# 3dimaging/rasr

Measured on AMD Instinct MI355X. Metric: frames/sec scored, 39-dim x 800k-density diag-GMM, higher is better.
Workload: dtype f32 (operands split into 2 f16 pieces, 3 f16 MFMA products, f32 accumulate); 1 GPU; 800k-density diag-GMM, 39-dim, diagonal-maximum, batched frames; scorer=diagonal-maximum, mixtures=5000, densities_per_mixture=160, covariance_tying=pooled, dimension=39, frames_per_launch=32768, parallelism=frame-sharded replicas x1

## Files before the change

include/rasr_gmm.h:

```cpp
#ifndef RASR_GMM_H
#define RASR_GMM_H

#include <stddef.h>
#include <stdint.h>

#ifdef __cplusplus
extern "C" {
#endif

#define GMM_OK 0
#define GMM_ERR_INVALID_ARGUMENT -1
#define GMM_ERR_UNSUPPORTED -2
#define GMM_ERR_DEVICE -3
#define GMM_ERR_OUT_OF_MEMORY -4
#define GMM_ERR_CAPACITY -5

typedef enum {
    GMM_BATCH_DIAGONAL_MAXIMUM_FLOAT = 0,
    GMM_BATCH_PRESELECTION_FLOAT     = 1,
    GMM_BATCH_PRESELECTION_INT       = 2,
    GMM_BATCH_DIAGONAL_MAXIMUM_INT   = 3,
    GMM_BATCH_DIAGONAL_MAXIMUM_FAST  = 4,
    GMM_DIAGONAL_MAXIMUM             = 5,
    GMM_SIMD_DIAGONAL_MAXIMUM        = 9,
// ... 26 lines not shown
    uint32_t clusters;
    uint32_t select_clusters;
    uint32_t clustering_iterations;
    float    backoff_score;
    const char* cache_archive;
} gmm_scorer_config;

#define GMM_FLAG_NATIVE_F32 1u
#define GMM_FLAG_SPLIT_TILE16 2u
#define GMM_FLAG_SPLIT_TILE32 4u
#define GMM_FLAG_REFERENCE_ORDER 8u
#define GMM_FLAG_FULL_KEYS 16u
#define GMM_FLAG_NO_SCORE_ONLY_TWIN 32u
#define GMM_FLAG_CACHE_ARCHIVE_READ_ONLY 64u
#define GMM_FLAG_ACCEPT_SPREAD_BOUND 128u

typedef struct gmm_scorer gmm_scorer;

void gmm_default_config(gmm_scorer_config* cfg);

int gmm_scorer_create(const gmm_mixture_set* mixture_set, gmm_scorer_type type,
                      const gmm_scorer_config* config, int device, gmm_scorer** out);
int gmm_scorer_destroy(gmm_scorer* scorer);

uint32_t gmm_scorer_n_mixtures(const gmm_scorer* scorer);
uint32_t gmm_scorer_dimension(const gmm_scorer* scorer);
uint32_t gmm_scorer_n_covariances(const gmm_scorer* scorer);
int      gmm_scorer_type_of(const gmm_scorer* scorer);

int gmm_score_device(gmm_scorer* scorer, const float* frames, uint32_t n_frames, uint32_t frame_stride,
// ... 43 lines not shown
                              double* log_z, double* minimum_score, uint32_t* minimum_index, uint32_t* n_active);

int gmm_host_alloc(size_t bytes, void** ptr);
int gmm_host_free(void* ptr);

int gmm_scorer_quantization(const gmm_scorer* scorer, float* scaling, float* inverse_quantization_factor);

int gmm_scorer_multiply_and_quantize(const gmm_scorer* scorer, const float* feature, uint8_t* out);

int gmm_prepare_quantized_host(const gmm_mixture_set* mixture_set, gmm_scorer_type type, float* scaling,
                               float* isv, float* log_norm, uint8_t* prepared_mean, int32_t* constant_weight);

int gmm_scorer_launch_info(const gmm_scorer* scorer, uint32_t n_frames, uint32_t* n_launches,
                           const char** main_kernel_name);

int gmm_scorer_k_steps(const gmm_scorer* scorer, uint32_t* k_steps);

int gmm_float_spread_bound(const gmm_mixture_set* mixture_set, gmm_scorer_type type, const gmm_scorer_config* config,
                           double* statistic, double* predicted);
int gmm_scorer_spread_bound(const gmm_scorer* scorer, double* statistic, double* predicted);

int gmm_scorer_set_timing(gmm_scorer* scorer, int enable);
int gmm_scorer_kernel_time(gmm_scorer* scorer, double* total_ms, uint32_t* n_launches, int reset);

#define GMM_CLUSTERING_BUILT 0
#define GMM_CLUSTERING_WRITTEN 1
#define GMM_CLUSTERING_CACHED 2
int gmm_scorer_clustering_source(const gmm_scorer* scorer, int* source);
int gmm_cache_archive_read_item(const char* path, const char* name, void* data, uint64_t capacity, uint64_t* size);
int gmm_cache_archive_write_item(const char* path, const char* name, const void* data, uint64_t size);
// ... 31 lines not shown
```

rasr_amd/_capi.py:

```python
from __future__ import annotations

import ctypes
import os

_HERE = os.path.dirname(os.path.abspath(__file__))
LIB_PATH = os.environ.get("RASR_GMM_LIB") or os.path.join(_HERE, "lib", "librasr_gmm.so")

GMM_OK = 0
GMM_ERR_INVALID_ARGUMENT = -1
GMM_ERR_UNSUPPORTED = -2
GMM_ERR_DEVICE = -3
GMM_ERR_OUT_OF_MEMORY = -4
GMM_ERR_CAPACITY = -5
GMM_ESTIMATOR_CHUNK = 512
STATE_POSTERIOR_CHUNK = 256
DEFAULT_WEIGHT_THRESHOLD = 2.0 ** -23
GMM_FLAG_NATIVE_F32 = 1
GMM_FLAG_SPLIT_TILE16 = 2
GMM_FLAG_SPLIT_TILE32 = 4
GMM_FLAG_REFERENCE_ORDER = 8
GMM_FLAG_FULL_KEYS = 16
GMM_FLAG_NO_SCORE_ONLY_TWIN = 32
GMM_FLAG_CACHE_ARCHIVE_READ_ONLY = 64
GMM_FLAG_ACCEPT_SPREAD_BOUND = 128
FLOAT_CONTRACT = 1e-4
GMM_CLUSTERING = {0: "built", 1: "written", 2: "cached"}

BATCH_DIAGONAL_MAXIMUM_FLOAT = 0
BATCH_PRESELECTION_FLOAT = 1
BATCH_PRESELECTION_INT = 2
BATCH_DIAGONAL_MAXIMUM_INT = 3
BATCH_DIAGONAL_MAXIMUM_FAST = 4
DIAGONAL_MAXIMUM = 5
SIMD_DIAGONAL_MAXIMUM = 9
DIAGONAL_SUM = 12

SCORER_TYPES = {
    "batch-diagonal-maximum-float": BATCH_DIAGONAL_MAXIMUM_FLOAT,
    "batch-diagonal-maximum-int": BATCH_DIAGONAL_MAXIMUM_INT,
# ... 97 lines not shown
      ctypes.c_double, ctypes.c_void_p, ctypes.c_void_p, ctypes.c_uint32, ctypes.c_void_p, ctypes.c_void_p,
      ctypes.c_void_p, ctypes.c_void_p, ctypes.c_void_p]),
    ("gmm_state_posteriors_host", ctypes.c_int,
     [ctypes.c_void_p, ctypes.c_void_p, ctypes.c_uint32, ctypes.c_uint32, ctypes.c_void_p, ctypes.c_double,
      ctypes.c_double, ctypes.c_void_p, ctypes.c_void_p, ctypes.c_uint32, ctypes.c_void_p, ctypes.c_void_p,
      ctypes.c_void_p, ctypes.c_void_p]),
    ("gmm_host_alloc", ctypes.c_int, [ctypes.c_size_t, ctypes.POINTER(ctypes.c_void_p)]),
    ("gmm_host_free", ctypes.c_int, [ctypes.c_void_p]),
    ("gmm_scorer_quantization", ctypes.c_int, [ctypes.c_void_p, _f32p, _f32p]),
    ("gmm_scorer_multiply_and_quantize", ctypes.c_int, [ctypes.c_void_p, ctypes.c_void_p, ctypes.c_void_p]),
    ("gmm_prepare_quantized_host", ctypes.c_int,
     [ctypes.POINTER(MixtureSetDesc), ctypes.c_int, _f32p, ctypes.c_void_p, ctypes.c_void_p, ctypes.c_void_p,
      ctypes.c_void_p]),
    ("gmm_scorer_launch_info", ctypes.c_int,
     [ctypes.c_void_p, ctypes.c_uint32, _u32p, ctypes.POINTER(ctypes.c_char_p)]),
    ("gmm_scorer_k_steps", ctypes.c_int, [ctypes.c_void_p, _u32p]),
    ("gmm_float_spread_bound", ctypes.c_int,
     [ctypes.POINTER(MixtureSetDesc), ctypes.c_int, ctypes.POINTER(ScorerConfig), _f64p, _f64p]),
    ("gmm_scorer_spread_bound", ctypes.c_int, [ctypes.c_void_p, _f64p, _f64p]),
    ("gmm_scorer_set_timing", ctypes.c_int, [ctypes.c_void_p, ctypes.c_int]),
    ("gmm_scorer_kernel_time", ctypes.c_int,
     [ctypes.c_void_p, ctypes.POINTER(ctypes.c_double), _u32p, ctypes.c_int]),
    ("gmm_scorer_density_clustering", ctypes.c_int,
     [ctypes.c_void_p, _u32p, _u32p, ctypes.c_void_p, ctypes.c_void_p]),
    ("gmm_scorer_cluster_selection", ctypes.c_int, [ctypes.c_void_p, ctypes.c_uint32, ctypes.c_void_p]),
    ("gmm_scorer_clustering_source", ctypes.c_int, [ctypes.c_void_p, ctypes.POINTER(ctypes.c_int)]),
    ("gmm_cache_archive_read_item", ctypes.c_int,
     [ctypes.c_char_p, ctypes.c_char_p, ctypes.c_void_p, ctypes.c_uint64, ctypes.POINTER(ctypes.c_uint64)]),
    ("gmm_cache_archive_write_item", ctypes.c_int, [ctypes.c_char_p, ctypes.c_char_p, ctypes.c_void_p, ctypes.c_uint64]),
    ("gmm_density_clustering_seeds", ctypes.c_int, [ctypes.c_uint32, ctypes.c_uint32, _u32p]),
# ... 93 lines not shown
```

rasr_amd/csrc/gmm_kernels.hh:

```
#pragma once

#include <hip/hip_runtime.h>

#include <cstdint>
#include <mutex>
#include <set>
#include <type_traits>
#include <utility>

namespace rasr_gmm {

enum class Kernel { I8Seg, I8Cls, I8Presel, Direct, SplitPair, SplitWide, SplitPresel, Split32, SplitSum, Split32Sum, F32 };
constexpr bool isSplitKernel(Kernel k) {
    return k == Kernel::SplitPair || k == Kernel::SplitWide || k == Kernel::SplitPresel || k == Kernel::Split32 ||
           k == Kernel::SplitSum || k == Kernel::Split32Sum;
}

template <int... N, class F>
bool dispatchInt(uint32_t v, std::integer_sequence<int, N...>, F&& f) {
    return ((v == uint32_t(N) ? (f(std::integral_constant<int, N>{}), true) : false) || ...);
}

inline hipError_t allowDynamicLds(const void* fn, int bytes) {
    static std::mutex                        mu;
// ... 84 lines not shown
#ifndef GMM_SPLIT_FPB
#define GMM_SPLIT_FPB 256
#endif
constexpr uint32_t kSplitFramesPerBlock = GMM_SPLIT_FPB;
constexpr uint32_t kSplitWaves          = kSplitFramesPerBlock / 64;
constexpr uint32_t kSplitMainWaves      = kSplitFramesPerBlock / (16 * kSplitNF);
#ifndef GMM_SPLIT_WIDE
#define GMM_SPLIT_WIDE 1
#endif
constexpr uint32_t splitWideFrames(uint32_t ks) {
    return GMM_SPLIT_WIDE && ks <= 4 ? 256u : 0u;
}

constexpr uint32_t kSplitWideChunkTiles = (1u << 22) / 5u - 16u;

constexpr uint32_t kSplitLimbs   = 4;
constexpr uint32_t kSplitXXLimbs = 3;
constexpr int kSplitXXExp[kSplitXXLimbs] = {15, 4, -7};
inline uint32_t splitKSteps(uint32_t dimension) {
    return (3 * dimension + kSplitLimbs + kSplitXXLimbs + 31) / 32;
}
inline uint32_t splitKSteps32(uint32_t dimension) {
    return (3 * dimension + kSplitLimbs + kSplitXXLimbs + 15) / 16;
}
inline uint32_t splitCovKSteps(uint32_t dimension) {
    return (6 * dimension + kSplitLimbs + 31) / 32;
}

struct SplitArgs {
    const void*     tileH;
// ... 3 lines not shown
    const float*    frameXX;
    const int32_t*  frameExp;
    float*          scores;
    uint32_t*       best;
    uint32_t        nFrames, nFramesPad, scoreStride;
    uint32_t        nChunks, nFrameTiles, mixBase;
    int             flavor;
    uint32_t        tileBits;
    float           offsetK0;
    float           outScale;
    const uint32_t* selT;
    const void*     tileClu;
    uint32_t        nClusters;
    int             presel;
    float           backoff;
};

hipError_t launchPrepareFramesI8(const float* frames, uint32_t nFrames, uint32_t frameStride, uint32_t nFramesPad,
                                 uint32_t nFramesRead, uint32_t D, uint32_t C, uint32_t KS, const float* isv, int8_t* frameQ,
                                 int32_t* frameSS, hipStream_t stream);
hipError_t launchPrepareFramesF32(const float* frames, uint32_t nFrames, uint32_t frameStride, uint32_t nFramesPad,
                                  uint32_t nFramesRead, uint32_t D, uint32_t C, uint32_t KS, int foldNorm, const float* isv,
                                  const float* centre, float* frameX,
                                  float* frameXX, hipStream_t stream);
hipError_t launchPrepareFramesSplit(const float* frames, uint32_t nFrames, uint32_t frameStride, uint32_t nFramesRead,
                                    uint32_t D, uint32_t rows, uint32_t kSteps, const float* isv, const float* centre,
                                    const float* dimScale,
                                    const int32_t* limbExp, void* frameH, float* frameXX, int32_t* frameExp,
                                    hipStream_t stream);
hipError_t launchPrepareFramesSplitCov(const float* frames, uint32_t nFrames, uint32_t frameStride, uint32_t nFramesRead,
// ... 120 lines not shown
```

rasr_amd/csrc/gmm_kernels_i8.hip:

```cpp
#include <type_traits>

#include "gmm_device.hh"

#ifndef GMM_I8_SLOTS
#define GMM_I8_SLOTS 1
#endif

namespace rasr_gmm {
namespace dev {

__global__ __launch_bounds__(256) void prepareFramesI8(const float* __restrict__ frames, uint32_t nFrames,
                                                        uint32_t frameStride, uint32_t nFramesPad,
                                                        uint32_t nFramesRead, uint32_t D,
                                                        uint32_t C, uint32_t KS, const float* __restrict__ isv,
                                                        int8_t* __restrict__ frameQ, int32_t* __restrict__ frameSS) {
    const uint32_t g = blockIdx.x * 8u + (threadIdx.x >> 5), blk = threadIdx.x & 31u;
    if (g >= C * nFramesRead)
        return;
    const uint32_t c = g / nFramesRead, f = g % nFramesRead;
    const float*   x  = frames + static_cast<size_t>(f) * frameStride;
    const float*   iv = isv + static_cast<size_t>(c) * KS * 64;
    i32x4*         out = reinterpret_cast<i32x4*>(frameQ + (static_cast<size_t>(c) * nFramesPad + f) * KS * 64);
    int            ss = 0;
    if (blk < KS * 4) {
// ... 1089 lines not shown
        if constexpr (KS == 1) {
            if (a.scoreOnly == 2) {
                constexpr int NFC = (W == 4 && NF == kI8NF) ? kI8ClsNF : NF;
                hipLaunchKernelGGL((dev::scoreI8Cls<NFC, kSeg, W>), dim3(grid), dim3(64 * W), 0, s, a, a.mixTileOff,
                                   a.scores, a.mixOddMask);
                return;
            }
            if (a.scoreOnly) {
                hipLaunchKernelGGL((dev::scoreI8Seg<NF, 1, false, kSeg, true, W>), dim3(grid), dim3(64 * W), 0, s, a,
                                   a.mixTileOff, a.scores, nullptr, a.mixOddMask);
                return;
            }
        }
        hipLaunchKernelGGL((dev::scoreI8Seg<NF, KS, false, kSeg, false, W>), dim3(grid), dim3(64 * W), 0, s, a,
                           a.mixTileOff, a.scores, a.best, nullptr);
        return;
    }
    hipLaunchKernelGGL((dev::scoreI8<NF, KS, MULTI>), dim3(grid), dim3(256), 0, s, a);
}

hipError_t launchScoreI8(const I8Args& a, uint32_t kSteps, bool multiCov, hipStream_t stream) {
    const uint32_t grid = 8u * ((a.nChunks + 7u) / 8u) * a.nFrameTiles;
    if (grid == 0)
        return hipSuccess;
    if (a.presel && (multiCov || a.nClusters == 0 || a.nClusters > 256 || !a.selT || !a.tileClu ||
                     (kI8PreselNF == 8 && !a.selC)))
        return hipErrorInvalidValue;
    if (a.scoreOnly && (multiCov || kSteps != 1 || !a.mixOddMask))
        return hipErrorInvalidValue;
    if (a.smallTile && a.presel)
        return hipErrorInvalidValue;
    if (kSteps == 1 && a.smallTile == 2 && !multiCov)
        launchI8T<4, 1, false, 1>(a, grid, stream);
// ... 17 lines not shown
```

rasr_amd/csrc/gmm_kernels_split.hip:

```cpp
#include "gmm_device.hh"

#include <type_traits>
#include <utility>

#ifndef GMM_SPLIT_MIN_WAVES
#define GMM_SPLIT_MIN_WAVES 1
#endif
#ifndef GMM_SPLIT_IL
#define GMM_SPLIT_IL 24
#endif
#ifndef GMM_SPLIT_PRESEL_NF
#define GMM_SPLIT_PRESEL_NF 8
#endif
constexpr int splitPreselNF(int ks) { return GMM_SPLIT_PRESEL_NF == 8 && ks <= 5 ? 8 : 4; }
#ifndef GMM_SPLIT_PF
#define GMM_SPLIT_PF 2
#endif
#ifndef GMM_SPLIT_SUM_NF
#define GMM_SPLIT_SUM_NF 4
#endif

namespace rasr_gmm {
namespace dev {

// ... 503 lines not shown
                }
            }
        });
    }
}

#ifndef GMM_SPLIT_WIDE_PF
#define GMM_SPLIT_WIDE_PF 3
#endif
#ifndef GMM_SPLIT_WIDE_IL
#define GMM_SPLIT_WIDE_IL 64
#endif
#define GMM_WIDE_ROW_RSRC(ptr) \
    __builtin_amdgcn_make_buffer_rsrc((ptr) + rowOff, (short)0, static_cast<int>(a.nFrames * 4u), 0x00020000)

template <int KS, bool BEST>
__global__ __launch_bounds__(64, 1) void scoreSplitWide(SplitArgs a, const uint32_t* __restrict__ mixTileOff) {
    constexpr uint32_t FPB = splitWideFrames(KS);
    constexpr int      NF = FPB / 16, NH = NF / 4, PF = GMM_SPLIT_WIDE_PF, U = PF % 2 == 0 ? PF : 2 * PF;
    static_assert(FPB == 256, "16 column blocks: the frame operands fill the accumulator file, four frames per lane");
    const int      lane = threadIdx.x & 63;
    const uint32_t g    = static_cast<uint32_t>(lane) >> 4;
    uint32_t       chunk, ft;
    if (!mapBlock(a.nChunks, a.nFrameTiles, chunk, ft))
        return;
    const uint32_t frame0 = ft * FPB, fb0 = frame0 / 16u;
    const uint32_t m0 = a.chunkMixOff[chunk], m1 = a.chunkMixOff[chunk + 1];
    const uint32_t T0 = mixTileOff[m0], T1 = mixTileOff[m1];

    const auto     tileRsrc = __builtin_amdgcn_make_buffer_rsrc(
            const_cast<char*>(static_cast<const char*>(a.tileH)) + static_cast<size_t>(T0) * (KS * 1024u), (short)0,
            static_cast<int>((T1 - T0 + PF) * (KS * 1024u)), 0x00020000);
    const uint32_t laneOff  = static_cast<uint32_t>(lane) * 16u;
    const auto     loadTile = [&](uint32_t tt, f16x8(&A)[KS]) __attribute__((always_inline)) {
        const uint32_t so = (tt - T0) * (KS * 1024u);
#pragma unroll
        for (int s = 0; s < KS; ++s)
            A[s] = __builtin_bit_cast(f16x8, __builtin_amdgcn_raw_buffer_load_b128(tileRsrc, laneOff + 1024u * s, so, 0));
    };
    const f16x8*   fh = static_cast<const f16x8*>(a.frameH);
// ... 17 lines not shown
            asm volatile("" : "+a"(B[cb][s]));
#pragma unroll
    for (int h = 0; h < NH; ++h)
        asm volatile("" ::"v"(eOut[h]));

    f16x8 R[PF][KS];
#pragma unroll
    for (int j = 0; j < PF; ++j)
        loadTile(T0 + j, R[j]);

    const uint32_t kmask = BEST ? (1u << a.tileBits) - 1u : 0u;
    uint32_t       vmask = ~kmask;
    asm volatile("" : "+v"(vmask));
    const float noneScore = __fmul_rn(a.outScale, a.flavor == 2 ? 0.5f * 3.40282347e+38f : 3.40282347e+38f);

    uint32_t   best[NF][2];
    const auto resetBest = [&]() {
#pragma unroll
        for (int cb = 0; cb < NF; ++cb)
            best[cb][0] = best[cb][1] = 0xffffffffu;
    };
    const auto chain = [&](const f16x8(&A)[KS], f32x4(&acc)[NF]) __attribute__((always_inline)) {
#pragma unroll
        for (int cb = 0; cb < NF; ++cb)
            acc[cb] = f32x4{0.0f, 0.0f, 0.0f, 0.0f};
#pragma unroll
        for (int s = 0; s < KS; ++s)
#pragma unroll
            for (int cb = 0; cb < NF; ++cb)
                acc[cb] = __builtin_amdgcn_mfma_f32_16x16x32_f16(A[s], B[cb][s], acc[cb], 0, 0, 0);
    };
    uint32_t   tag[4] = {0u, 1u, 2u, 3u};
    const auto epilogue = [&](const f32x4(&acc)[NF]) __attribute__((always_inline)) {
#pragma unroll
        for (int r = 0; r < 4; ++r)
            asm("" : "+s"(tag[r]));
#pragma unroll
        for (int cb = 0; cb < NF; ++cb) {
            uint32_t v[4];
#pragma unroll
            for (int r = 0; r < 4; ++r)
                v[r] = BEST ? (__float_as_uint(acc[cb][r]) & vmask) | tag[r] : __float_as_uint(acc[cb][r]);
            best[cb][0] = umin3(umin3(best[cb][0], v[0], v[1]), v[2], v[3]);
        }
#pragma unroll
        for (int r = 0; r < 4; ++r)
            tag[r] += 4u;
    };

    uint32_t   m = m0, tEnd = m0 < m1 ? mixTileOff[m0 + 1] : T0;
    uint32_t tNxt  = mixTileOff[min(m0 + 2u, m1)];
    size_t rowOff  = static_cast<size_t>(m0 - a.mixBase) * a.scoreStride;
    const auto nextMixture = [&](uint32_t tNext) __attribute__((always_inline)) {
        ++m;
        rowOff += a.scoreStride;
        tEnd = m < m1 ? tNxt : tNext;
        tNxt = mixTileOff[min(m + 2u, m1)];
    };
    const auto emit = [&]() __attribute__((always_inline)) {
        uint32_t key[NH], idx[NH];
        float    score[NH];
#pragma unroll
        for (int h = 0; h < NH; ++h) {
            uint32_t k[4], grp;
#pragma unroll
            for (int cb = 0; cb < 4; ++cb)
                k[cb] = min(best[4 * h + cb][0], best[4 * h + cb][1]);
            reduceKeysSplit<BEST>(k, key[h], grp);
            idx[h] = (((key[h] & kmask & ~3u) | grp) << 2) | (key[h] & 3u);
        }
        finalizeSplit<BEST, NH>(a, key, kmask, eOut, noneScore, score, idx);
        const uint32_t off = (frame0 + NH * static_cast<uint32_t>(lane)) * 4u;
        __builtin_amdgcn_raw_buffer_store_b128(u32x4{__float_as_uint(score[0]), __float_as_uint(score[1]),
                                                     __float_as_uint(score[2]), __float_as_uint(score[3])},
                                               GMM_WIDE_ROW_RSRC(a.scores), off, 0, GMM_STORE_CPOL);
        if constexpr (BEST)
            __builtin_amdgcn_raw_buffer_store_b128(u32x4{idx[0], idx[1], idx[2], idx[3]}, GMM_WIDE_ROW_RSRC(a.best), off, 0,
                                                   GMM_STORE_CPOL);
    };
    const auto advance = [&](uint32_t tNext) __attribute__((always_inline)) {
        nextMixture(tNext);
        while (m < m1 && tEnd == tNext) {
// ... 2 lines not shown
        }
    };
    const auto finish = [&](uint32_t tNext) __attribute__((always_inline)) {
        if (__builtin_expect(tNext == tEnd, 0)) {
            emit();
            resetBest();
            advance(tNext);
#pragma unroll
            for (int r = 0; r < 4; ++r)
                tag[r] &= 3u;
        }
    };
    constexpr int  kIl   = GMM_SPLIT_WIDE_IL * NF / 16;
    constexpr int  kIlE  = 3 * NF;
    constexpr bool kTail = kIl >= kIlE && kIlE + KS + 4 <= NF * KS;
    const auto    step = [&](const f16x8(&A)[KS], f32x4(&cur)[NF], const f32x4(&prev)[NF]) __attribute__((always_inline)) {
        chain(A, cur);
        epilogue(prev);
#pragma unroll
        for (int i = 0; i < (kTail ? kIlE : kIl); ++i) {
            __builtin_amdgcn_sched_group_barrier(0x008, 1, 0);
            __builtin_amdgcn_sched_group_barrier(0x002, 2, 0);
        }
        if constexpr (kTail) {
#pragma unroll
            for (int i = 0; i < KS; ++i) {
                __builtin_amdgcn_sched_group_barrier(0x008, 1, 0);
                __builtin_amdgcn_sched_group_barrier(0x020, 1, 0);
            }
#pragma unroll
            for (int i = 0; i < 4; ++i) {
                __builtin_amdgcn_sched_group_barrier(0x008, 1, 0);
                __builtin_amdgcn_sched_group_barrier(0x004, 2, 0);
            }
            __builtin_amdgcn_sched_group_barrier(0x008, NF * KS - kIlE - KS - 4, 0);
        }
        else
            __builtin_amdgcn_sched_group_barrier(0x008, NF * KS - kIl, 0);
    };

    resetBest();
    while (m < m1 && tEnd == T0) {
        emit();
        nextMixture(T0);
    }
    if (T0 < T1) {
        f32x4 acc[2][NF];
        chain(R[0], acc[0]);
        loadTile(T0 + PF, R[0]);
        uint32_t t = T0 + 1;
        const auto sub = [&](auto ic, uint32_t tt) __attribute__((always_inline)) {
            constexpr int i = decltype(ic)::value, set = (1 + i) % PF, cur = (1 + i) % 2, prv = i % 2;
            step(R[set], acc[cur], acc[prv]);
            loadTile(tt + PF, R[set]);
            finish(tt);
        };
        for (; t + U <= T1; t += U)
            staticFor<U>([&](auto ic) __attribute__((always_inline)) { sub(ic, t + decltype(ic)::value); });
        bool live = true;
        staticFor<U>([&](auto ic) __attribute__((always_inline)) {
            constexpr int  i  = decltype(ic)::value;
            const uint32_t tt = t + i;
            if (live) {
                if (tt < T1) {
                    sub(ic, tt);
// ... 738 lines not shown
}

hipError_t launchPrepareFramesSplitCov(const float* frames, uint32_t nFrames, uint32_t frameStride, uint32_t nFramesRead,
                                       uint32_t D, uint32_t kSteps, const float* centre, const float* dimScale,
                                       const int32_t* limbExp, void* frameH, int32_t* frameExp, hipStream_t stream) {
    hipLaunchKernelGGL(dev::prepareFramesSplitCov, dim3((nFramesRead + 7) / 8), dim3(256), 0, stream, frames, nFrames,
                       frameStride, nFramesRead, D, kSteps, centre, dimScale, limbExp, static_cast<dev::u32x4*>(frameH),
                       frameExp);
    return hipGetLastError();
}

template <int KS>
static void launchSplitK(const SplitArgs& a, Kernel kernel, uint32_t grid, hipStream_t s) {
    if constexpr (splitWideFrames(KS) != 0) {
        if (kernel == Kernel::SplitWide) {
            hipLaunchKernelGGL((a.best ? dev::scoreSplitWide<KS, true> : dev::scoreSplitWide<KS, false>), dim3(grid), dim3(64),
                               0, s, a, a.mixTileOff);
            return;
        }
    }
    if (kernel == Kernel::SplitPresel) {
        const uint32_t lds = kSplitFramesPerBlock / 64u * a.nClusters * 64u;
        (void)allowDynamicLds(reinterpret_cast<const void*>(&dev::scoreSplit<KS, false, true>),
                              static_cast<int>(kSplitFramesPerBlock / 64u * 256u * 64u));
        hipLaunchKernelGGL((dev::scoreSplit<KS, false, true>), dim3(grid), dim3(kSplitFramesPerBlock / splitPreselNF(KS) * 4),
                           lds, s, a, a.mixTileOff);
    }
    else
        hipLaunchKernelGGL((a.best ? dev::scoreSplit<KS, true, false> : dev::scoreSplit<KS, false, false>), dim3(grid),
                           dim3(64 * kSplitMainWaves), 0, s, a, a.mixTileOff);
}

// ... 12 lines not shown
template <int KS>
static void launchSplit32SumK(const SplitArgs& a, uint32_t grid, hipStream_t s) {
    hipLaunchKernelGGL((a.best ? dev::scoreSplit32Sum<KS, true> : dev::scoreSplit32Sum<KS, false>), dim3(grid),
                       dim3(64 * (kSplitFramesPerBlock / 128)), 0, s, a, a.mixTileOff);
}

using KSteps16 = std::integer_sequence<int, 8, 7, 6, 5, 4, 3, 2, 1>;
using KSteps32 = std::integer_sequence<int, 10, 9, 8, 7, 6, 5, 4, 3, 2, 1>;

hipError_t launchScoreSplit(const SplitArgs& a, Kernel kernel, uint32_t kSteps16, hipStream_t stream) {
    const uint32_t grid = 8u * ((a.nChunks + 7u) / 8u) * a.nFrameTiles;
    if (grid == 0)
        return hipSuccess;
    if ((a.presel != 0) != (kernel == Kernel::SplitPresel) ||
        (a.presel && (a.nClusters == 0 || a.nClusters > 256 || !a.selT || !a.tileClu)) ||
        (kernel == Kernel::SplitWide && splitWideFrames(kSteps16) == 0))
        return hipErrorInvalidValue;
    bool ok = false;
    switch (kernel) {
        case Kernel::Split32:
            ok = dispatchInt(kSteps16, KSteps32{}, [&](auto ks) { launchSplit32K<decltype(ks)::value>(a, grid, stream); });
            break;
        case Kernel::SplitPair:
        case Kernel::SplitWide:
        case Kernel::SplitPresel:
            ok = dispatchInt(kSteps16, KSteps16{}, [&](auto ks) { launchSplitK<decltype(ks)::value>(a, kernel, grid, stream); });
            break;
        case Kernel::Split32Sum:
            ok = dispatchInt(kSteps16, KSteps32{}, [&](auto ks) { launchSplit32SumK<decltype(ks)::value>(a, grid, stream); });
            break;
        case Kernel::SplitSum:
// ... 9 lines not shown
```

rasr_amd/csrc/gmm_score.cc:

```cpp
#include <algorithm>
#include <cstdlib>

#include "gmm_scorer.hh"

namespace rasr_gmm {


KernelPlan kernelPlanOf(const gmm_scorer& s) {
    const bool presel = isPreselection(s.type);
    KernelPlan p;
    p.launches = presel ? 3 : 2;
    if (const auto* q = s.quantized()) {
        p.kernel = presel ? Kernel::I8Presel : (q->scoreOnly == kScoreOnlySlots ? Kernel::I8Cls : Kernel::I8Seg);
        p.framesPerBlock = presel ? kI8PreselFramesPerBlock
                                  : (p.kernel == Kernel::I8Cls ? kI8ClsFramesPerBlock : kI8FramesPerBlock);
        p.smallTiles     = !presel;
        p.name           = "scoreI8";
    }
    else if (std::holds_alternative<DirectModel>(s.model))
        p = {Kernel::Direct, kDirectFramesPerBlock, false, p.launches, "scoreDirect"};
    else if (const auto* m = std::get_if<SplitModel>(&s.model)) {
        const bool     rows32 = m->splitRows == 32;
        const uint32_t wide   = splitWideFrames(m->kSteps16);
        p.framesPerBlock      = kSplitFramesPerBlock;
// ... 31 lines not shown
    return p;
}

int waitAsync(gmm_scorer* s) {
    if (!s->host.asyncCall)
        return GMM_OK;
    s->host.asyncCall  = 0;
    const hipError_t e = hipEventSynchronize(s->host.asyncDone.get());
    if (e != hipSuccess)
        return fail(GMM_ERR_DEVICE, std::string("hipEventSynchronize (GMM_HOST_ASYNC call): ") + hipGetErrorString(e));
    return GMM_OK;
}

namespace {

int chunkTableFor(gmm_scorer* s, uint32_t nFrameTiles, const ChunkTable** out) {
    auto it = s->chunks.find(nFrameTiles);
    if (it != s->chunks.end()) {
        *out = &it->second;
        return GMM_OK;
    }
#ifndef GMM_TARGET_BLOCKS
#define GMM_TARGET_BLOCKS 8192
#endif
#ifndef GMM_SPLIT_TARGET_BLOCKS
#define GMM_SPLIT_TARGET_BLOCKS 2048
#endif
    static const uint32_t kOverride = [] {
        const char* e = std::getenv("RASR_GMM_TARGET_BLOCKS");
        const long  v = e ? std::strtol(e, nullptr, 10) : 0;
        return v > 0 ? static_cast<uint32_t>(v) : 0u;
    }();
    const Kernel   k       = s->plan.kernel;
    const uint32_t kTargetBlocks =
            kOverride ? kOverride
            : isSplitKernel(k) ? std::clamp<uint32_t>(nFrameTiles * 256u, 1024u,
                                             k == Kernel::SplitSum ? uint32_t(GMM_TARGET_BLOCKS)
                                                                   : uint32_t(GMM_SPLIT_TARGET_BLOCKS))
            : k == Kernel::I8Seg || k == Kernel::I8Cls ? std::clamp<uint32_t>(nFrameTiles * 1024u, 2048u, uint32_t(GMM_TARGET_BLOCKS))
                                                       : uint32_t(GMM_TARGET_BLOCKS);
    uint32_t target = std::max<uint32_t>(1, (kTargetBlocks + nFrameTiles - 1) / nFrameTiles);
    if (target > 8)
        target = (target + 7u) / 8u * 8u;
    target                  = std::min<uint32_t>(target, std::max<uint32_t>(1, s->nMix));
    uint32_t perChunk = std::max<uint32_t>(1, (s->nTiles + target - 1) / target);
    const uint32_t chunkCap = k == Kernel::SplitWide ? kSplitWideChunkTiles : 0xffffffffu;
    perChunk                = std::min(perChunk, chunkCap / 2u);
    std::vector<uint32_t> off{0};
    uint32_t              acc = 0;
    for (uint32_t m = 0; m < s->nMix; ++m) {
        acc += s->mixTileOff[m + 1] - s->mixTileOff[m];
        if (acc > chunkCap)
            return fail(GMM_ERR_CAPACITY, "a mixture has more tiles than a scoreSplitWide chunk can address");
        if (acc >= perChunk && m + 1 < s->nMix) {
            off.push_back(m + 1);
            acc = 0;
        }
    }
    off.push_back(s->nMix);
    ChunkTable ct;
    ct.nChunks = static_cast<uint32_t>(off.size() - 1);
    int rc     = upload(ct.dMixOff, off);
    if (rc != GMM_OK)
        return rc;
    *out = &s->chunks.emplace(nFrameTiles, std::move(ct)).first->second;
    return GMM_OK;
}

struct TimedSpan {
    gmm_scorer* s;
    hipStream_t stream;
    hipEvent_t  e = nullptr;
    hipError_t begin() {
        if (!s->timing)
            return hipSuccess;
        if (s->eventsUsed == s->events.size()) {
            std::pair<Event, Event> ev;
            hipError_t              err = ev.first.create();
// ... 122 lines not shown
    a.tileH       = m.dTileH.get();
    a.frameH      = m.dFrameH.get();
    a.frameXX     = m.dFrameXX.get();
    a.frameExp    = m.dFrameExp.get();
    a.best        = s.flavor != Flavor::BatchFloat ? c.best : nullptr;
    a.flavor      = s.flavor == Flavor::DiagonalMaximum ? 2 : (s.flavor == Flavor::DiagonalSum ? 4 : 3);
    a.tileBits    = m.keyBits;
    a.offsetK0    = m.offsetK0;
    a.presel      = c.plan.kernel == Kernel::SplitPresel ? 1 : 0;
    if (s.presel) {
        a.selT      = s.presel->dSelT.get();
        a.tileClu   = s.presel->dTileClu.get();
        a.nClusters = s.presel->clustering.nClusters;
    }
    a.backoff = s.cfg.backoff_score;
    return launchScoreSplit(a, c.plan.kernel, m.kSteps16, c.stream);
}

hipError_t prepareFrames(const gmm_scorer& s, const F32Model& m, const Call& c) {
    return launchPrepareFramesF32(c.frames, c.nFrames, c.frameStride, s.nFramesPad, c.plan.nFramesRead, s.D, s.C, m.kSteps,
                                  m.foldNorm ? 1 : 0, s.dIsv.get(), m.dCentre.get(), m.dFrameX.get(), m.dFrameXX.get(),
                                  c.stream);
}

hipError_t launch(const gmm_scorer& s, const F32Model& m, const Call& c) {
    F32Args a = argsOf<F32Args>(s, c);
    a.tileA       = static_cast<const float*>(m.dTileA.get());
    a.tileCov     = m.dTileCov.get();
    a.rowDns      = m.dRowDns.get();
    a.frameX      = m.dFrameX.get();
    a.frameXX     = m.dFrameXX.get();
// ... 44 lines not shown

int gmm_score_device(gmm_scorer* s, const float* frames, uint32_t nFrames, uint32_t frameStride, float* scores,
                     uint32_t* best, uint32_t scoreStride, void* stream) {
    if (!s)
        return fail(GMM_ERR_INVALID_ARGUMENT, "null scorer");
    const int wrc = waitAsync(s);
    if (wrc != GMM_OK)
        return wrc;
    return scoreImpl(s, frames, nFrames, frameStride, scores, best, scoreStride, static_cast<hipStream_t>(stream));
}

int gmm_scorer_launch_info(const gmm_scorer* s, uint32_t nFrames, uint32_t* nLaunches, const char** name) {
    if (!s)
        return fail(GMM_ERR_INVALID_ARGUMENT, "null scorer");
    s = modelOf(s);
    (void)nFrames;
    if (nLaunches)
        *nLaunches = s->plan.launches;
    if (name)
        *name = s->plan.name;
    return GMM_OK;
}

int gmm_scorer_k_steps(const gmm_scorer* s, uint32_t* kSteps) {
    if (!s || !kSteps)
        return fail(GMM_ERR_INVALID_ARGUMENT, "null scorer or output");
    s = modelOf(s);
    if (const auto* q = s->quantized())
        *kSteps = q->kSteps;
    else if (const auto* m = std::get_if<SplitModel>(&s->model))
        *kSteps = m->kSteps16;
    else if (const auto* f = std::get_if<F32Model>(&s->model))
        *kSteps = f->kSteps;
    else if (const auto* d = std::get_if<DirectModel>(&s->model))
        *kSteps = (d->L - 4u) / 4u;
// ... 7 lines not shown
```

rasr_amd/csrc/gmm_scorer.hh:

```
#pragma once

#include <hip/hip_runtime.h>

#include <map>
#include <memory>
#include <string>
#include <type_traits>
#include <utility>
#include <variant>
#include <vector>

#include "../../include/rasr_gmm.h"
#include "gmm_hostio.hh"
#include "gmm_kernels.hh"
#include "gmm_prepare.hh"
#include "gmm_presel.hh"

namespace rasr_gmm {

void setLastError(const std::string& msg);

inline int fail(int code, const std::string& msg) {
    setLastError(msg);
    return code;
// ... 77 lines not shown
    uint32_t    launches       = 2;
    const char* name           = "scoreF32";
};

struct LaunchPlan {
    Kernel   kernel;
    uint32_t framesPerBlock;
    int      smallTile;
    uint32_t nFrameTiles, nFramesRead;
};


struct ChunkTable {
    uint32_t               nChunks = 0;
    DeviceBuffer<uint32_t> dMixOff;
};

struct QuantizedModel {
    uint32_t kSteps = 0, idxBits = 1, paddedDimension = 0;
    int      scoreOnly = kScoreOnlyNone;
    float    scaling = 0, scalingSquared = 0, invQ = 0, batchScale = 0;
    std::vector<float>     isvScaled;
    DeviceBuffer<void>     dTileA, dTileP;
    DeviceBuffer<uint32_t> dTileCov, dMixOddMask;
    DeviceBuffer<int8_t>   dFrameQ;
    DeviceBuffer<int32_t>  dFrameSS;
};

struct SplitModel {
    uint32_t kSteps16 = 0;
// ... 88 lines not shown
    using Flavor = rasr_gmm::Flavor;
    gmm_scorer_type   type;
    Flavor            flavor;
    int               device = 0;
    gmm_scorer_config cfg{};
    uint32_t          D = 0, C = 0, nMix = 0, mixBase = 0;
    uint32_t          nMixSet = 0;
    uint32_t          nTiles = 0;
    uint32_t          nFramesPad = 0;
    double            spreadStat = 0, spreadPredicted = 0;
    std::vector<uint32_t>            mixTileOff;
    rasr_gmm::DeviceBuffer<uint32_t> dMixTileOff;
    rasr_gmm::DeviceBuffer<float>    dIsv;
    rasr_gmm::KernelPlan             plan;
    std::map<uint32_t, rasr_gmm::ChunkTable> chunks;
    bool                                                   timing = false;
    std::vector<std::pair<rasr_gmm::Event, rasr_gmm::Event>> events;
    size_t                                                 eventsUsed = 0;
    std::variant<std::monostate, rasr_gmm::QuantizedModel, rasr_gmm::SplitModel, rasr_gmm::F32Model,
                 rasr_gmm::DirectModel>
            model;
    std::unique_ptr<rasr_gmm::Preselection> presel;
    std::unique_ptr<rasr_gmm::PairTables>   pairs;
    std::unique_ptr<rasr_gmm::StateScratch> state;
    rasr_gmm::HostPipeline                  host;
    std::unique_ptr<rasr_gmm::DensityGroup, rasr_gmm::DensityGroupDelete> group;
    std::unique_ptr<gmm_scorer> scoresOnly;
    std::string cacheArchive;

    const rasr_gmm::QuantizedModel* quantized() const { return std::get_if<rasr_gmm::QuantizedModel>(&model); }
// ... 39 lines not shown
```

rasr_amd/scorer.py:

```python
from __future__ import annotations

import ctypes
import os

import numpy as np

from . import _capi
from .mixture_set import MixtureSet


def _type_id(t) -> int:
    if isinstance(t, str):
        return _capi.SCORER_TYPES[t]
    return int(t)


def default_config() -> _capi.ScorerConfig:
    cfg = _capi.ScorerConfig()
    _capi.load_library().gmm_default_config(ctypes.byref(cfg))
    return cfg


class Scorer:

    def __init__(self, mixture_set: MixtureSet, scorer_type="SIMD-diagonal-maximum", max_frames: int = 4096,
                 device: int = 0, mixture_weight_scale: float = 1.0, gaussian_scale: float = 1.0,
                 score_scale: float = 1.0, mixture_range: tuple[int, int] | None = None, native_f32: bool = False,
                 split_tile16: bool = False, split_tile32: bool = False, clusters: int = 256,
                 select_clusters: int = 32, clustering_iterations: int = 5, backoff_score: float = 40000.0,
                 reference_order: bool = False, devices=None, exchange: str = "auto", full_keys: bool = False,
                 no_score_only_twin: bool = False, cache_archive: str | None = None,
                 cache_archive_read_only: bool = False, accept_spread_bound: bool = False):
        self._lib = _capi.load_library()
        self.mixture_set = mixture_set
        self.type = _type_id(scorer_type)
        cfg = default_config()
        cfg.max_frames = int(max_frames)
        cfg.mixture_weight_scale = mixture_weight_scale
        cfg.gaussian_scale = gaussian_scale
        cfg.score_scale = score_scale
        if native_f32:
            cfg.flags |= _capi.GMM_FLAG_NATIVE_F32
        if split_tile16:
            cfg.flags |= _capi.GMM_FLAG_SPLIT_TILE16
        if split_tile32:
            cfg.flags |= _capi.GMM_FLAG_SPLIT_TILE32
        if reference_order:
            cfg.flags |= _capi.GMM_FLAG_REFERENCE_ORDER
        if full_keys:
            cfg.flags |= _capi.GMM_FLAG_FULL_KEYS
        if no_score_only_twin:
            cfg.flags |= _capi.GMM_FLAG_NO_SCORE_ONLY_TWIN
        if accept_spread_bound:
            cfg.flags |= _capi.GMM_FLAG_ACCEPT_SPREAD_BOUND
        cfg.clusters = int(clusters)
        cfg.select_clusters = int(select_clusters)
        cfg.clustering_iterations = int(clustering_iterations)
        cfg.backoff_score = float(backoff_score)
        self._cache_archive = None if cache_archive is None else os.fsencode(cache_archive)
        cfg.cache_archive = self._cache_archive
        if cache_archive_read_only:
            cfg.flags |= _capi.GMM_FLAG_CACHE_ARCHIVE_READ_ONLY
        if mixture_range is not None:
            cfg.mixture_begin, cfg.mixture_end = int(mixture_range[0]), int(mixture_range[1])
        self.max_frames = int(max_frames)
        self._mixture_range = ((int(cfg.mixture_begin), int(cfg.mixture_end)) if cfg.mixture_end
                            else (0, int(len(mixture_set.mixture_offsets)) - 1))
        self._desc = mixture_set.desc()
        h = ctypes.c_void_p()
# ... 23 lines not shown
        try:
            self.close()
        except Exception:
            pass

    @property
    def handle(self):
        return self._h

    def main_kernel(self) -> str:
        n = ctypes.c_uint32()
        name = ctypes.c_char_p()
        _capi.check(self._lib.gmm_scorer_launch_info(self._h, 1, ctypes.byref(n), ctypes.byref(name)),
                    "gmm_scorer_launch_info")
        return name.value.decode()

    def k_steps(self) -> int:
        k = ctypes.c_uint32()
        _capi.check(self._lib.gmm_scorer_k_steps(self._h, ctypes.byref(k)), "gmm_scorer_k_steps")
        return k.value

    def spread_bound(self) -> tuple[float, float]:
        st, pr = ctypes.c_double(), ctypes.c_double()
        _capi.check(self._lib.gmm_scorer_spread_bound(self._h, ctypes.byref(st), ctypes.byref(pr)),
                    "gmm_scorer_spread_bound")
        return st.value, pr.value

    def density_clustering(self):
        n = ctypes.c_uint32()
        dp = ctypes.c_uint32()
# ... 309 lines not shown
```

Baseline: 7.989 million frames/s.

## Specialize split-wide kernel for chunks with uniform per-mixture tile counts

```diff
diff --git a/include/rasr_gmm.h b/include/rasr_gmm.h
--- a/include/rasr_gmm.h
+++ b/include/rasr_gmm.h
@@ -64,6 +64,7 @@
 #define GMM_FLAG_NO_SCORE_ONLY_TWIN 32u
 #define GMM_FLAG_CACHE_ARCHIVE_READ_ONLY 64u
 #define GMM_FLAG_ACCEPT_SPREAD_BOUND 128u
+#define GMM_FLAG_SPLIT_WIDE_GENERIC 256u
 
 typedef struct gmm_scorer gmm_scorer;
 
@@ -137,6 +138,10 @@
 int gmm_scorer_launch_info(const gmm_scorer* scorer, uint32_t n_frames, uint32_t* n_launches,
                            const char** main_kernel_name);
 
+int gmm_scorer_chunk_forms(gmm_scorer* scorer, uint32_t n_frames, uint32_t* n_uniform, uint32_t* n_generic);
+
+int gmm_scorer_set_chunk_target(gmm_scorer* scorer, uint32_t target_blocks);
+
 int gmm_scorer_k_steps(const gmm_scorer* scorer, uint32_t* k_steps);
 
 int gmm_float_spread_bound(const gmm_mixture_set* mixture_set, gmm_scorer_type type, const gmm_scorer_config* config,
diff --git a/rasr_amd/_capi.py b/rasr_amd/_capi.py
--- a/rasr_amd/_capi.py
+++ b/rasr_amd/_capi.py
@@ -23,6 +23,7 @@
 GMM_FLAG_NO_SCORE_ONLY_TWIN = 32
 GMM_FLAG_CACHE_ARCHIVE_READ_ONLY = 64
 GMM_FLAG_ACCEPT_SPREAD_BOUND = 128
+GMM_FLAG_SPLIT_WIDE_GENERIC = 256
 FLOAT_CONTRACT = 1e-4
 GMM_CLUSTERING = {0: "built", 1: "written", 2: "cached"}
 
@@ -150,6 +151,8 @@
       ctypes.c_void_p]),
     ("gmm_scorer_launch_info", ctypes.c_int,
      [ctypes.c_void_p, ctypes.c_uint32, _u32p, ctypes.POINTER(ctypes.c_char_p)]),
+    ("gmm_scorer_chunk_forms", ctypes.c_int, [ctypes.c_void_p, ctypes.c_uint32, _u32p, _u32p]),
+    ("gmm_scorer_set_chunk_target", ctypes.c_int, [ctypes.c_void_p, ctypes.c_uint32]),
     ("gmm_scorer_k_steps", ctypes.c_int, [ctypes.c_void_p, _u32p]),
     ("gmm_float_spread_bound", ctypes.c_int,
      [ctypes.POINTER(MixtureSetDesc), ctypes.c_int, ctypes.POINTER(ScorerConfig), _f64p, _f64p]),
diff --git a/rasr_amd/csrc/gmm_kernels.hh b/rasr_amd/csrc/gmm_kernels.hh
--- a/rasr_amd/csrc/gmm_kernels.hh
+++ b/rasr_amd/csrc/gmm_kernels.hh
@@ -122,6 +122,16 @@
 
 constexpr uint32_t kSplitWideChunkTiles = (1u << 22) / 5u - 16u;
 
+constexpr uint32_t kSplitWideUniformKSteps = 4;
+using SplitWideUniformT = std::integer_sequence<int, 10, 8>;
+template <int... N>
+constexpr bool splitWideUniformTIn(uint32_t t, std::integer_sequence<int, N...>) {
+    return ((t == uint32_t(N)) || ...);
+}
+constexpr bool splitWideUniformT(uint32_t ks, uint32_t t) {
+    return GMM_SPLIT_WIDE && ks == kSplitWideUniformKSteps && splitWideUniformTIn(t, SplitWideUniformT{});
+}
+
 constexpr uint32_t kSplitLimbs   = 4;
 constexpr uint32_t kSplitXXLimbs = 3;
 constexpr int kSplitXXExp[kSplitXXLimbs] = {15, 4, -7};
@@ -155,6 +165,8 @@
     uint32_t        nClusters;
     int             presel;
     float           backoff;
+    const uint32_t* chunkList;
+    uint32_t        uniformT;
 };
 
 hipError_t launchPrepareFramesI8(const float* frames, uint32_t nFrames, uint32_t frameStride, uint32_t nFramesPad,
diff --git a/rasr_amd/csrc/gmm_kernels_i8.hip b/rasr_amd/csrc/gmm_kernels_i8.hip
--- a/rasr_amd/csrc/gmm_kernels_i8.hip
+++ b/rasr_amd/csrc/gmm_kernels_i8.hip
@@ -1127,9 +1127,9 @@
         }
         hipLaunchKernelGGL((dev::scoreI8Seg<NF, KS, false, kSeg, false, W>), dim3(grid), dim3(64 * W), 0, s, a,
                            a.mixTileOff, a.scores, a.best, nullptr);
-        return;
-    }
-    hipLaunchKernelGGL((dev::scoreI8<NF, KS, MULTI>), dim3(grid), dim3(256), 0, s, a);
+    }
+    else
+        hipLaunchKernelGGL((dev::scoreI8<NF, KS, MULTI>), dim3(grid), dim3(256), 0, s, a);
 }
 
 hipError_t launchScoreI8(const I8Args& a, uint32_t kSteps, bool multiCov, hipStream_t stream) {
diff --git a/rasr_amd/csrc/gmm_kernels_split.hip b/rasr_amd/csrc/gmm_kernels_split.hip
--- a/rasr_amd/csrc/gmm_kernels_split.hip
+++ b/rasr_amd/csrc/gmm_kernels_split.hip
@@ -1,5 +1,6 @@
 #include "gmm_device.hh"
 
+#include <numeric>
 #include <type_traits>
 #include <utility>
 
@@ -541,7 +542,7 @@
 #define GMM_WIDE_ROW_RSRC(ptr) \
     __builtin_amdgcn_make_buffer_rsrc((ptr) + rowOff, (short)0, static_cast<int>(a.nFrames * 4u), 0x00020000)
 
-template <int KS, bool BEST>
+template <int KS, bool BEST, int T>
 __global__ __launch_bounds__(64, 1) void scoreSplitWide(SplitArgs a, const uint32_t* __restrict__ mixTileOff) {
     constexpr uint32_t FPB = splitWideFrames(KS);
     constexpr int      NF = FPB / 16, NH = NF / 4, PF = GMM_SPLIT_WIDE_PF, U = PF % 2 == 0 ? PF : 2 * PF;
@@ -551,6 +552,8 @@
     uint32_t       chunk, ft;
     if (!mapBlock(a.nChunks, a.nFrameTiles, chunk, ft))
         return;
+    if (a.chunkList)
+        chunk = a.chunkList[chunk];
     const uint32_t frame0 = ft * FPB, fb0 = frame0 / 16u;
     const uint32_t m0 = a.chunkMixOff[chunk], m1 = a.chunkMixOff[chunk + 1];
     const uint32_t T0 = mixTileOff[m0], T1 = mixTileOff[m1];
@@ -598,11 +601,11 @@
     asm volatile("" : "+v"(vmask));
     const float noneScore = __fmul_rn(a.outScale, a.flavor == 2 ? 0.5f * 3.40282347e+38f : 3.40282347e+38f);
 
-    uint32_t   best[NF][2];
+    uint32_t   best[NF];
     const auto resetBest = [&]() {
 #pragma unroll
         for (int cb = 0; cb < NF; ++cb)
-            best[cb][0] = best[cb][1] = 0xffffffffu;
+            best[cb] = 0xffffffffu;
     };
     const auto chain = [&](const f16x8(&A)[KS], f32x4(&acc)[NF]) __attribute__((always_inline)) {
 #pragma unroll
@@ -625,11 +628,22 @@
 #pragma unroll
             for (int r = 0; r < 4; ++r)
                 v[r] = BEST ? (__float_as_uint(acc[cb][r]) & vmask) | tag[r] : __float_as_uint(acc[cb][r]);
-            best[cb][0] = umin3(umin3(best[cb][0], v[0], v[1]), v[2], v[3]);
+            best[cb] = umin3(umin3(best[cb], v[0], v[1]), v[2], v[3]);
         }
 #pragma unroll
         for (int r = 0; r < 4; ++r)
             tag[r] += 4u;
+    };
+    const auto epilogueAt = [&](auto pos, const f32x4(&acc)[NF]) __attribute__((always_inline)) {
+#pragma unroll
+        for (int cb = 0; cb < NF; ++cb) {
+            uint32_t v[4];
+#pragma unroll
+            for (int r = 0; r < 4; ++r)
+                v[r] = BEST ? (__float_as_uint(acc[cb][r]) & vmask) | ((static_cast<uint32_t>(decltype(pos)::value) << 2) | r)
+                            : __float_as_uint(acc[cb][r]);
+            best[cb] = umin3(umin3(best[cb], v[0], v[1]), v[2], v[3]);
+        }
     };
 
     uint32_t   m = m0, tEnd = m0 < m1 ? mixTileOff[m0 + 1] : T0;
@@ -649,7 +663,7 @@
             uint32_t k[4], grp;
 #pragma unroll
             for (int cb = 0; cb < 4; ++cb)
-                k[cb] = min(best[4 * h + cb][0], best[4 * h + cb][1]);
+                k[cb] = best[4 * h + cb];
             reduceKeysSplit<BEST>(k, key[h], grp);
             idx[h] = (((key[h] & kmask & ~3u) | grp) << 2) | (key[h] & 3u);
         }
@@ -682,9 +696,7 @@
     constexpr int  kIl   = GMM_SPLIT_WIDE_IL * NF / 16;
     constexpr int  kIlE  = 3 * NF;
     constexpr bool kTail = kIl >= kIlE && kIlE + KS + 4 <= NF * KS;
-    const auto    step = [&](const f16x8(&A)[KS], f32x4(&cur)[NF], const f32x4(&prev)[NF]) __attribute__((always_inline)) {
-        chain(A, cur);
-        epilogue(prev);
+    const auto    stepSchedule = [&]() __attribute__((always_inline)) {
 #pragma unroll
         for (int i = 0; i < (kTail ? kIlE : kIl); ++i) {
             __builtin_amdgcn_sched_group_barrier(0x008, 1, 0);
@@ -706,6 +718,11 @@
         else
             __builtin_amdgcn_sched_group_barrier(0x008, NF * KS - kIl, 0);
     };
+    const auto step = [&](const f16x8(&A)[KS], f32x4(&cur)[NF], const f32x4(&prev)[NF]) __attribute__((always_inline)) {
+        chain(A, cur);
+        epilogue(prev);
+        stepSchedule();
+    };
 
     resetBest();
     while (m < m1 && tEnd == T0) {
@@ -717,6 +734,28 @@
         chain(R[0], acc[0]);
         loadTile(T0 + PF, R[0]);
         uint32_t t = T0 + 1;
+        if constexpr (T != 0) {
+            constexpr int      L = U / std::gcd(U, T) * T, MB = L / T;
+            const uint32_t     nBody = (T1 - T0 - 1u) / L;
+            for (uint32_t b = 0; b < nBody; ++b, t += L)
+                staticFor<L>([&](auto kc) __attribute__((always_inline)) {
+                    constexpr int k = decltype(kc)::value, i = k % U, set = (1 + i) % PF, cur = (1 + i) % 2, prv = i % 2;
+                    chain(R[set], acc[cur]);
+                    epilogueAt(std::integral_constant<int, k % T>{}, acc[prv]);
+                    stepSchedule();
+                    loadTile(t + k + PF, R[set]);
+                    __builtin_amdgcn_sched_barrier(0);
+                    if constexpr (k % T == T - 1) {
+                        emit();
+                        resetBest();
+                        rowOff += a.scoreStride;
+                        __builtin_amdgcn_sched_barrier(0);
+                    }
+                });
+            m += nBody * MB;
+            tEnd = mixTileOff[m + 1];
+            tNxt = mixTileOff[min(m + 2u, m1)];
+        }
         const auto sub = [&](auto ic, uint32_t tt) __attribute__((always_inline)) {
             constexpr int i = decltype(ic)::value, set = (1 + i) % PF, cur = (1 + i) % 2, prv = i % 2;
             step(R[set], acc[cur], acc[prv]);
@@ -1485,8 +1524,16 @@
 static void launchSplitK(const SplitArgs& a, Kernel kernel, uint32_t grid, hipStream_t s) {
     if constexpr (splitWideFrames(KS) != 0) {
         if (kernel == Kernel::SplitWide) {
-            hipLaunchKernelGGL((a.best ? dev::scoreSplitWide<KS, true> : dev::scoreSplitWide<KS, false>), dim3(grid), dim3(64),
-                               0, s, a, a.mixTileOff);
+            bool uniform = false;
+            if constexpr (KS == kSplitWideUniformKSteps)
+                uniform = dispatchInt(a.uniformT, SplitWideUniformT{}, [&](auto tc) {
+                    constexpr int T = decltype(tc)::value;
+                    hipLaunchKernelGGL((a.best ? dev::scoreSplitWide<KS, true, T> : dev::scoreSplitWide<KS, false, T>),
+                                       dim3(grid), dim3(64), 0, s, a, a.mixTileOff);
+                });
+            if (!uniform)
+                hipLaunchKernelGGL((a.best ? dev::scoreSplitWide<KS, true, 0> : dev::scoreSplitWide<KS, false, 0>), dim3(grid),
+                                   dim3(64), 0, s, a, a.mixTileOff);
             return;
         }
     }
@@ -1529,7 +1576,8 @@
         return hipSuccess;
     if ((a.presel != 0) != (kernel == Kernel::SplitPresel) ||
         (a.presel && (a.nClusters == 0 || a.nClusters > 256 || !a.selT || !a.tileClu)) ||
-        (kernel == Kernel::SplitWide && splitWideFrames(kSteps16) == 0))
+        (kernel == Kernel::SplitWide && splitWideFrames(kSteps16) == 0) ||
+        (a.uniformT != 0 && (kernel != Kernel::SplitWide || !splitWideUniformT(kSteps16, a.uniformT))))
         return hipErrorInvalidValue;
     bool ok = false;
     switch (kernel) {
diff --git a/rasr_amd/csrc/gmm_score.cc b/rasr_amd/csrc/gmm_score.cc
--- a/rasr_amd/csrc/gmm_score.cc
+++ b/rasr_amd/csrc/gmm_score.cc
@@ -69,6 +69,33 @@
 
 namespace {
 
+int splitWideParts(const gmm_scorer& s, const std::vector<uint32_t>& off, ChunkTable& ct) {
+    const auto*    model   = std::get_if<SplitModel>(&s.model);
+    const bool     generic = (s.cfg.flags & GMM_FLAG_SPLIT_WIDE_GENERIC) != 0 || !model;
+    std::map<uint32_t, std::vector<uint32_t>> byT;
+    for (uint32_t c = 0; c + 1 < off.size(); ++c) {
+        uint32_t T = generic ? 0u : s.mixTileOff[off[c] + 1] - s.mixTileOff[off[c]];
+        for (uint32_t m = off[c]; T != 0 && m < off[c + 1]; ++m)
+            if (s.mixTileOff[m + 1] - s.mixTileOff[m] != T)
+                T = 0;
+        if (T != 0 && !splitWideUniformT(model->kSteps16, T))
+            T = 0;
+        byT[T].push_back(c);
+    }
+    for (auto& [T, list] : byT) {
+        ChunkTable::Part part;
+        part.uniformT = T;
+        part.nChunks  = static_cast<uint32_t>(list.size());
+        if (byT.size() > 1) {
+            const int rc = upload(part.dList, list);
+            if (rc != GMM_OK)
+                return rc;
+        }
+        ct.parts.push_back(std::move(part));
+    }
+    return GMM_OK;
+}
+
 int chunkTableFor(gmm_scorer* s, uint32_t nFrameTiles, const ChunkTable** out) {
     auto it = s->chunks.find(nFrameTiles);
     if (it != s->chunks.end()) {
@@ -88,7 +115,8 @@
     }();
     const Kernel   k       = s->plan.kernel;
     const uint32_t kTargetBlocks =
-            kOverride ? kOverride
+            s->chunkTarget ? s->chunkTarget
+            : kOverride    ? kOverride
             : isSplitKernel(k) ? std::clamp<uint32_t>(nFrameTiles * 256u, 1024u,
                                              k == Kernel::SplitSum ? uint32_t(GMM_TARGET_BLOCKS)
                                                                    : uint32_t(GMM_SPLIT_TARGET_BLOCKS))
@@ -117,6 +145,8 @@
     ct.nChunks = static_cast<uint32_t>(off.size() - 1);
     int rc     = upload(ct.dMixOff, off);
     if (rc != GMM_OK)
+        return rc;
+    if (k == Kernel::SplitWide && (rc = splitWideParts(*s, off, ct)) != GMM_OK)
         return rc;
     *out = &s->chunks.emplace(nFrameTiles, std::move(ct)).first->second;
     return GMM_OK;
@@ -269,7 +299,17 @@
         a.nClusters = s.presel->clustering.nClusters;
     }
     a.backoff = s.cfg.backoff_score;
-    return launchScoreSplit(a, c.plan.kernel, m.kSteps16, c.stream);
+    if (c.ct->parts.empty())
+        return launchScoreSplit(a, c.plan.kernel, m.kSteps16, c.stream);
+    for (const ChunkTable::Part& part : c.ct->parts) {
+        a.nChunks   = part.nChunks;
+        a.chunkList = part.dList.get();
+        a.uniformT  = part.uniformT;
+        const hipError_t e = launchScoreSplit(a, c.plan.kernel, m.kSteps16, c.stream);
+        if (e != hipSuccess)
+            return e;
+    }
+    return hipSuccess;
 }
 
 hipError_t prepareFrames(const gmm_scorer& s, const F32Model& m, const Call& c) {
@@ -344,11 +384,52 @@
     if (!s)
         return fail(GMM_ERR_INVALID_ARGUMENT, "null scorer");
     s = modelOf(s);
-    (void)nFrames;
-    if (nLaunches)
-        *nLaunches = s->plan.launches;
+    if (nLaunches) {
+        const auto it = s->chunks.find(planFor(*s, std::max(nFrames, 1u)).nFrameTiles);
+        const size_t parts = it != s->chunks.end() ? it->second.parts.size() : 0;
+        *nLaunches = s->plan.launches + static_cast<uint32_t>(parts > 1 ? parts - 1 : 0);
+    }
     if (name)
         *name = s->plan.name;
+    return GMM_OK;
+}
+
+int gmm_scorer_set_chunk_target(gmm_scorer* s, uint32_t targetBlocks) {
+    if (!s)
+        return fail(GMM_ERR_INVALID_ARGUMENT, "null scorer");
+    const int wrc = waitAsync(s);
+    if (wrc != GMM_OK)
+        return wrc;
+    for (gmm_scorer* p : s->group ? partsOf(s) : std::vector<gmm_scorer*>{s}) {
+        GMM_HIP_CHECK(hipSetDevice(p->device));
+        GMM_HIP_CHECK(hipDeviceSynchronize());
+        p->chunkTarget = targetBlocks;
+        p->chunks.clear();
+    }
+    return GMM_OK;
+}
+
+int gmm_scorer_chunk_forms(gmm_scorer* s, uint32_t nFrames, uint32_t* nUniform, uint32_t* nGeneric) {
+    if (!s)
+        return fail(GMM_ERR_INVALID_ARGUMENT, "null scorer");
+    uint32_t uniform = 0, generic = 0;
+    for (gmm_scorer* p : s->group ? partsOf(s) : std::vector<gmm_scorer*>{s}) {
+        if (p->nMix == 0)
+            continue;
+        GMM_HIP_CHECK(hipSetDevice(p->device));
+        const ChunkTable* ct = nullptr;
+        const int         rc = chunkTableFor(p, planFor(*p, std::max(nFrames, 1u)).nFrameTiles, &ct);
+        if (rc != GMM_OK)
+            return rc;
+        if (ct->parts.empty())
+            generic += ct->nChunks;
+        for (const ChunkTable::Part& part : ct->parts)
+            (part.uniformT ? uniform : generic) += part.nChunks;
+    }
+    if (nUniform)
+        *nUniform = uniform;
+    if (nGeneric)
+        *nGeneric = generic;
     return GMM_OK;
 }
 
diff --git a/rasr_amd/csrc/gmm_scorer.hh b/rasr_amd/csrc/gmm_scorer.hh
--- a/rasr_amd/csrc/gmm_scorer.hh
+++ b/rasr_amd/csrc/gmm_scorer.hh
@@ -115,6 +115,12 @@
 struct ChunkTable {
     uint32_t               nChunks = 0;
     DeviceBuffer<uint32_t> dMixOff;
+    struct Part {
+        uint32_t               uniformT = 0;
+        uint32_t               nChunks  = 0;
+        DeviceBuffer<uint32_t> dList;
+    };
+    std::vector<Part> parts;
 };
 
 struct QuantizedModel {
@@ -233,6 +239,7 @@
     rasr_gmm::DeviceBuffer<float>    dIsv;
     rasr_gmm::KernelPlan             plan;
     std::map<uint32_t, rasr_gmm::ChunkTable> chunks;
+    uint32_t          chunkTarget = 0;
     bool                                                   timing = false;
     std::vector<std::pair<rasr_gmm::Event, rasr_gmm::Event>> events;
     size_t                                                 eventsUsed = 0;
diff --git a/rasr_amd/scorer.py b/rasr_amd/scorer.py
--- a/rasr_amd/scorer.py
+++ b/rasr_amd/scorer.py
@@ -30,7 +30,8 @@
                  select_clusters: int = 32, clustering_iterations: int = 5, backoff_score: float = 40000.0,
                  reference_order: bool = False, devices=None, exchange: str = "auto", full_keys: bool = False,
                  no_score_only_twin: bool = False, cache_archive: str | None = None,
-                 cache_archive_read_only: bool = False, accept_spread_bound: bool = False):
+                 cache_archive_read_only: bool = False, accept_spread_bound: bool = False,
+                 split_wide_generic: bool = False):
         self._lib = _capi.load_library()
         self.mixture_set = mixture_set
         self.type = _type_id(scorer_type)
@@ -53,6 +54,8 @@
             cfg.flags |= _capi.GMM_FLAG_NO_SCORE_ONLY_TWIN
         if accept_spread_bound:
             cfg.flags |= _capi.GMM_FLAG_ACCEPT_SPREAD_BOUND
+        if split_wide_generic:
+            cfg.flags |= _capi.GMM_FLAG_SPLIT_WIDE_GENERIC
         cfg.clusters = int(clusters)
         cfg.select_clusters = int(select_clusters)
         cfg.clustering_iterations = int(clustering_iterations)
@@ -106,6 +109,15 @@
         _capi.check(self._lib.gmm_scorer_launch_info(self._h, 1, ctypes.byref(n), ctypes.byref(name)),
                     "gmm_scorer_launch_info")
         return name.value.decode()
+
+    def chunk_forms(self, n_frames: int = 1) -> tuple[int, int]:
+        u, g = ctypes.c_uint32(), ctypes.c_uint32()
+        _capi.check(self._lib.gmm_scorer_chunk_forms(self._h, int(n_frames), ctypes.byref(u), ctypes.byref(g)),
+                    "gmm_scorer_chunk_forms")
+        return u.value, g.value
+
+    def set_chunk_target(self, target_blocks: int) -> None:
+        _capi.check(self._lib.gmm_scorer_set_chunk_target(self._h, int(target_blocks)), "gmm_scorer_set_chunk_target")
 
     def k_steps(self) -> int:
         k = ctypes.c_uint32()
```

After: 8.093 million frames/s, median of 6. +1.3%, better.
